# nima-siboni/collectivecrossing

Hardware: NVIDIA B200
Metric: agent_steps_per_sec (higher is better)
Workload: dtype u8 (lattice cells, flag bytes; int32 step counters); rewards: f64 products rounded once to f32

## Files before the change

### __graft_entry__.py

```python

from __future__ import annotations

import sys
from pathlib import Path

ROOT = Path(__file__).resolve().parent
for p in (str(ROOT), str(ROOT / "tests")):
    if p not in sys.path:
        sys.path.insert(0, p)


def build() -> None:
    from collectivecrossing_b200 import _native

    from collectivecrossing_b200 import _abi

    _native.build(force=True)
    lib = _native.library()
    assert lib.cc_abi_version() == _abi.ABI_VERSION
    import oracle
    from oracle import stage_ref

    oracle.build(force=True)
    oracle.lib()
    stage_ref.stage()
    _write_sass()
    import collectivecrossing_b200


def _write_sass() -> None:
    import re
    import subprocess
    from collections import Counter

    from collectivecrossing_b200 import _native

    out_dir = ROOT / "profiles" / "sass"
    out_dir.mkdir(parents=True, exist_ok=True)
    wanted = {"cc_step_tpe2_kernel_8_fp32_b5": r"cc_step_tpe2_kernelILi8ELi4ELi5E", "cc_step_tpe2_kernel_8_int8_b5": r"cc_step_tpe2_kernelILi8ELi1ELi5E",
              "cc_step_tpe2_kernel_8_table_b5": r"cc_step_tpe2_kernelILi8ELi16ELi5E", "cc_step_tpe2_kernel_8_none_b5": r"cc_step_tpe2_kernelILi8ELi0ELi5E",
              "cc_step_tpe_kernel_8_fp32": r"cc_step_tpe_kernelILi8ELi4E", "cc_kernel_32_2_int8_step": r"cc_kernelILi32ELi2ELi1ELi0E"}
    try:
        dump = subprocess.run(["cuobjdump", "-sass", str(_native.LIB_PATH)], capture_output=True, text=True, check=True).stdout
    except Exception as exc:
        print(f"SASS dump skipped: {exc}")
        return
    for stale in out_dir.glob("*.sass"):
        stale.unlink()
    parts = re.split(r"(?=\n\s*Function : )", dump)
    counts = {}
    for name, pat in wanted.items():
        body = next((q for q in parts if re.search(r"Function : \S*" + pat, q)), None)
        if body is None:
            continue
        lines = [f"{m.group(1)}  {m.group(2).strip()}" for m in re.finditer(r"^\s+/\*([0-9a-f]{4,6})\*/\s+(.*?;)\s+/\*", body, flags=re.M)]
        head = body.strip().splitlines()[0]
        (out_dir / f"{name}.sass").write_text(head + "\n" + "\n".join(lines) + "\n")
        ops = Counter(re.sub(r"^@!?U?P\w+\s+", "", ln.split("  ", 1)[1]).split()[0].rstrip(";") for ln in lines)
        counts[name] = {"instructions": sum(ops.values()), "top": dict(ops.most_common(25)),
                        "tma": {k: v for k, v in ops.items() if k.startswith(("UBLKCP", "UTMA", "SYNCS"))}}
    import json

    (out_dir / "mnemonic_counts.json").write_text(json.dumps(counts, indent=1) + "\n")
    log = ROOT / "collectivecrossing_b200" / "csrc" / "ptxas.log"
    if log.exists():
        rows, name = [], None
        for ln in log.read_text().splitlines():
            m = re.search(r"Function properties for (\S+)", ln)
            if m:
                name = m.group(1)
            elif name and "bytes stack frame" in ln:
                stack = ln.strip()
            elif name and "Used" in ln and "registers" in ln:
                rows.append(f"{name}\n    {ln.split(':', 1)[1].strip()}; {stack}")
                name = None
        (out_dir / "ptxas_summary.txt").write_text("\n".join(sorted(set(rows))) + "\n")


def smoke() -> None:
    import numpy as np
    import torch
    from cases import readme_config

    import oracle
    from collectivecrossing_b200 import BatchedCollectiveCrossing, _abi
    from collectivecrossing_b200.lowering import lower_config

    cfg = readme_config(max_steps=20)
    n = 2048
    env = BatchedCollectiveCrossing(cfg, n, "cuda:0", seed=3, obs_dtype="float32", auto_reset=True, with_info=True)
    orc = oracle.OracleEnvs(lower_config(cfg), n, seed=3)
    env.reset()
    orc.reset()
    for t in range(30):
        out = env.step(policy="greedy")
        res = orc.step(policy="greedy", auto_reset=True, obs_dtype=_abi.OBS_FP32)
    torch.cuda.synchronize()
    env.check_error()
    assert np.array_equal(env.x.cpu().numpy(), orc.x) and np.array_equal(env.y.cpu().numpy(), orc.y)
    assert np.array_equal(env.flags.cpu().numpy(), orc.flags) and np.array_equal(env.step_count.cpu().numpy(), orc.step_count)
    assert np.array_equal(out.obs.cpu().numpy(), res["obs"]) and np.array_equal(out.reward.cpu().numpy(), res["reward"])
    assert np.array_equal(out.agent_flags.cpu().numpy(), res["agent_flags"]) and np.array_equal(out.env_flags.cpu().numpy(), res["env_flags"])
    st = env.stats()
    assert st["episodes"] == orc.stats.episodes > 0
    traj = env.rollout_trajectory(8, policy="greedy")
    for t in range(8):
        res = orc.step(policy="greedy", auto_reset=True, obs_dtype=_abi.OBS_FP32)
        assert np.array_equal(traj["obs"][t].cpu().numpy(), res["obs"]) and np.array_equal(traj["reward"][t].cpu().numpy(), res["reward"])
        assert np.array_equal(traj["agent_flags"][t].cpu().numpy(), res["agent_flags"]) and np.array_equal(traj["env_flags"][t].cpu().numpy(), res["env_flags"])
    assert np.array_equal(env.x.cpu().numpy(), orc.x) and np.array_equal(env.flags.cpu().numpy(), orc.flags)
    env.set_host_expand(2)
    host = env.make_host_buffers()
    env.step_host(host, policy="greedy")
    res = orc.step(policy="greedy", auto_reset=True, obs_dtype=_abi.OBS_FP32)
    assert np.array_equal(host["obs"].numpy(), res["obs"]) and np.array_equal(host["reward"].numpy(), res["reward"])
    assert np.array_equal(host["env_flags"].numpy(), res["env_flags"]) and env.last_host_call()["expand_threads"] == 1
    env.check_error()
    print(f"smoke ok: {n} envs x 39 steps, {st['episodes']} episodes, {env.launch_count} kernel launches "
          f"({env.last_kernel} mapping), bit-exact vs oracle")


if __name__ == "__main__":
# ... 3 lines not shown
```

### collectivecrossing_b200/csrc/cc_kernel_tpe2.cuh

```cuda
#pragma once
#include "cc_kernel_tpe.cuh"

#ifndef CCB_T2_MIN_BLOCKS
#define CCB_T2_MIN_BLOCKS 6
#endif

namespace ccb {

constexpr int kT2Warps = 4;
constexpr int kT2Threads = kT2Warps * 32;
constexpr int kT2MaxRows = 16, kT2MaxCols = 32, kT2MaxCells = 256;
constexpr int kT2BitmapBytesPerWarp = kT2MaxRows * 128;

enum { kT2InTram = 1u << 5, kT2AtDoor = 1u << 6, kT2Arrived = 1u << 7, kT2Valid = 1u << 28, kT2SpawnExcluded = 1u << 29 };

struct T2Tables {
    uint2 tab[2 * kT2MaxCells];
    uint8_t act2[kPolicyRows * 16];
    int dcell[8];
};
static_assert(sizeof(T2Tables) % 16 == 0, "copied as 16-byte vectors");

template <int A, int OBS>
struct T2Layout {
    static constexpr bool kImage = OBS == CC_OBS_INT8;
    static constexpr int kEnvBytes = A * (6 + 4 * A);
    static constexpr int kImageBytes = kImage ? 32 * kEnvBytes : 0;
    using L1 = TpeLayout<A, CC_OBS_FP32>;
    static constexpr bool kRows32 = OBS == CC_OBS_FP32;
    static constexpr int kRows32Bytes = kRows32 ? L1::kStageBytesPerWarp : 0;
    static constexpr bool kDirtyBitmap = kImage || kRows32;
    static constexpr int kBitmapOffset = kRows32 ? L1::kTplBytesPerWarp : 0;
    static constexpr int kBytesNeeded = kImage ? kImageBytes : (kRows32 ? kRows32Bytes : 0);
    static constexpr int kBytesPerWarp = kBytesNeeded > kBitmapOffset + kT2BitmapBytesPerWarp ? kBytesNeeded : kBitmapOffset + kT2BitmapBytesPerWarp;
    static constexpr int kDynBytes = kT2Warps * kBytesPerWarp;
};

__device__ __forceinline__ unsigned t2_fill(unsigned w, int k) {
    unsigned r;
    asm("prmt.b32 %0, %1, %2, %3;" : "=r"(r) : "r"(w), "r"(0u), "r"(0x8888u | ((unsigned)k * 0x1111u)));
    return r;
}
template <int B>
__device__ __forceinline__ unsigned t2_gather4(unsigned a, unsigned b, unsigned c, unsigned d) {
    const unsigned lo = __byte_perm(a, b, (unsigned)(B | ((4 + B) << 4)));
    const unsigned hi = __byte_perm(c, d, (unsigned)(B | ((4 + B) << 4)));
    return __byte_perm(lo, hi, 0x5410u);
}
template <int A, int B>
__device__ __forceinline__ void t2_gather(const uint2 (&e)[A], unsigned (&w)[2]) {
    auto g = [&](int k) { return e[k < A ? k : A - 1].x; };
    w[0] = t2_gather4<B>(g(0), g(1), g(2), g(3));
    w[1] = A > 4 ? t2_gather4<B>(g(4), g(5), g(6), g(7)) : 0u;
}
template <int A, bool STREAM>
__device__ __forceinline__ void t2_store_packed(void *base, int env, unsigned w0, unsigned w1) {
    unsigned char *q = static_cast<unsigned char *>(base) + (size_t)env * A;
    if constexpr (A == 8) {
        if constexpr (STREAM) __stcs(reinterpret_cast<uint2 *>(q), make_uint2(w0, w1));
        else *reinterpret_cast<uint2 *>(q) = make_uint2(w0, w1);
    } else if constexpr (A == 4) {
        if constexpr (STREAM) __stcs(reinterpret_cast<unsigned *>(q), w0);
        else *reinterpret_cast<unsigned *>(q) = w0;
    } else {
#pragma unroll
        for (int k = 0; k < A; ++k) q[k] = (unsigned char)((k < 4 ? w0 : w1) >> (8 * (k & 3)));
    }
}

#ifdef CCB_WITH_T2_TABLES
__global__ void __launch_bounds__(256) cc_t2_tables_kernel(const __grid_constant__ KParams p, T2Tables *out) {
    const int PW = p.W + 3, PH = p.H + 3;
    uint2 *tab = out->tab;
    uint8_t *act2 = out->act2;
    int *dcell = out->dcell;
    for (int i = threadIdx.x; i < 2 * kT2MaxCells; i += blockDim.x) {
        const int cell = i >> 1, type = i & 1;
        const int yy = cell / PW - 1, xx = cell - (yy + 1) * PW - 1;
        unsigned geo = 0;
        float rew = 0.f;
        if (cell < PW * PH && xx >= 0 && xx <= p.W && yy >= 0 && yy <= p.H) {
            const unsigned xv = make_xt(p, xx), yv = make_yt(p, type, yy);
            const unsigned u = xv + yv, f = (xv & yv) >> 24;
            const bool in_tram = f & 1u, at_door = f & 2u, arrived = f & 8u;
            const unsigned right = valid_position(p, xx + 1, yy), up = valid_position(p, xx, yy + 1), left = valid_position(p, xx - 1, yy),
                           down = valid_position(p, xx, yy - 1);
            geo = (u & 31u) | (in_tram ? kT2InTram : 0u) | (at_door ? kT2AtDoor : 0u) | (arrived ? kT2Arrived : 0u) | ((unsigned)xx << 8) |
                  ((unsigned)yy << 16) | ((right | (up << 1) | (left << 2) | (down << 3)) << 20) | ((left | (up << 1) | (right << 2) | (down << 3)) << 24) |
                  (valid_position(p, xx, yy) ? kT2Valid : 0u) | ((p.DL <= xx && xx <= p.DR && yy == p.D - 1) ? kT2SpawnExcluded : 0u);
            const bool boarding = type == 0;
            switch (p.reward_kind) {
            case CC_REWARD_DEFAULT:
                if (arrived) rew = p.rpf[0];
                else if (boarding) rew = at_door ? p.rpf[1] : (in_tram ? p.rpf[2] : (float)((double)(-(abs(xx - p.DC) + (p.D - yy))) * p.rp[3]));
                else rew = !in_tram ? p.rpf[2] : (float)((double)(abs(xx - p.DC) + (yy - p.D)) * p.rp[3]);
                break;
            case CC_REWARD_SIMPLE_DISTANCE: rew = (float)((double)(-abs(yy - (boarding ? p.YB : p.YE))) * p.rp[0]); break;
            case CC_REWARD_BINARY: rew = p.rpf[1]; break;
            default: rew = p.rpf[0]; break;
            }
        } else {
            geo = ((unsigned)min(max(xx, 0), p.W) << 8) | ((unsigned)min(max(yy, 0), p.H) << 16);
        }
        tab[i] = make_uint2(geo, __float_as_uint(rew));
    }
    for (int i = threadIdx.x; i < kPolicyRows * 16; i += blockDim.x) {
        const unsigned m = (unsigned)i & 15u;
        act2[i] = (uint8_t)greedy_decision(i >> 4, ((m >> 2) & 1u) | (m & 2u) | ((m & 1u) << 2) | (m & 8u));
    }
    if (threadIdx.x < 8) dcell[threadIdx.x] = threadIdx.x == 0 ? 1 : (threadIdx.x == 1 ? PW : (threadIdx.x == 2 ? -1 : (threadIdx.x == 3 ? -PW : 0)));
}
#endif

template <int A, int OBS, int BT>
__global__ void __launch_bounds__(kT2Threads, CCB_T2_MIN_BLOCKS) cc_step_tpe2_kernel(const __grid_constant__ KParams p) {
    using L = T2Layout<A, OBS>;
    const int B = BT >= 0 ? BT : p.B;
    static_assert(A >= 1 && A <= 8, "thread-per-env mapping is for crews of at most 8");
    static_assert(OBS == CC_OBS_NONE || OBS == CC_OBS_TABLE || (OBS == CC_OBS_INT8 && A == 8) || (OBS == CC_OBS_FP32 && A % 2 == 0),
                  "int8 rows: 8 agents; float32 rows: even crews (an env's block must be whole 16-byte vectors for the bulk copies)");
    static_assert(!L::kRows32 || L::L1::kTma, "float32 rows leave through the TMA image ring");
    constexpr unsigned kOnes = 0x01010101u;
    constexpr unsigned kM0 = A >= 4 ? kOnes : (kOnes >> (8 * (4 - A)));
    constexpr unsigned kM1 = A <= 4 ? 0u : (A == 8 ? kOnes : (kOnes >> (8 * (8 - A))));
    extern __shared__ __align__(16) unsigned char smem[];
    __shared__ __align__(16) T2Tables tb;
    __shared__ unsigned long long red_all[kT2Warps * kStCount];

    const int lane = threadIdx.x & 31, warp = threadIdx.x >> 5;
    const int PW = p.W + 3, PH = p.H + 3;

    for (int i = threadIdx.x; i < (int)(sizeof(T2Tables) / 16); i += blockDim.x)
        reinterpret_cast<uint4 *>(&tb)[i] = static_cast<const uint4 *>(p.t2_tables)[i];
    const int n_warps = (int)blockDim.x >> 5;
    for (int i = threadIdx.x; i < n_warps * L::kBytesPerWarp / 4; i += blockDim.x) reinterpret_cast<unsigned *>(smem)[i] = 0u;
    __shared__ __align__(16) unsigned lut[L::kRows32 ? L::L1::kLutWords : 4];
    if constexpr (L::kRows32) {
        __syncthreads();
        using L1 = typename L::L1;
        for (int w = threadIdx.x; w < L1::kLutWords; w += blockDim.x) {
            const int src = w < L1::PPE ? tpe_source<A>(w / L1::R, w % L1::R) : kSrcM;
            lut[w] = src >= 0 ? (unsigned)(src * L1::PSZ) : (0x80000000u | (unsigned)(-src));
        }
        float2 *t = reinterpret_cast<float2 *>(smem + warp * L::kBytesPerWarp + lane * L1::TSB);
        t[2 * A] = make_float2((float)p.DC, (float)p.D); t[2 * A + 1] = make_float2((float)p.DL, (float)p.DR); t[2 * A + 2] = make_float2(-1.f, -1.f);
    }
    const TpeConstPairs kc = {make_uint2(__float_as_uint((float)p.DC), __float_as_uint((float)p.D)),
                              make_uint2(__float_as_uint((float)p.DL), __float_as_uint((float)p.DR)),
                              make_uint2(__float_as_uint(-1.f), __float_as_uint(-1.f))};
    unsigned long long *red = red_all + warp * kStCount;
    if (lane < kStCount) red[lane] = 0ull;
    if (blockIdx.x == 0 && threadIdx.x == 0) *p.tpe_counter_next = 0u;
    __syncthreads();

    const unsigned tab_s = (unsigned)__cvta_generic_to_shared(tb.tab), act_s = (unsigned)__cvta_generic_to_shared(tb.act2),
                   dc_s = (unsigned)__cvta_generic_to_shared(tb.dcell);
    unsigned char *wsmem = smem + warp * L::kBytesPerWarp;
    const unsigned img_s = (unsigned)__cvta_generic_to_shared(wsmem);
    const unsigned bm = img_s + (unsigned)L::kBitmapOffset + 4u * lane;
    unsigned tbase[A];
#pragma unroll
    for (int k = 0; k < A; ++k) tbase[k] = tab_s + (k < B ? 0u : 8u);
    unsigned boardw[2];
    boardw[0] = (B >= 4 ? kOnes : (B <= 0 ? 0u : (kOnes >> (8 * (4 - B))))) & kM0;
    boardw[1] = (B <= 4 ? 0u : (B >= 8 ? kOnes : (kOnes >> (8 * (8 - B))))) & kM1;
    const unsigned typew0 = kM0 & ~boardw[0], typew1 = kM1 & ~boardw[1];

    auto lookup = [&](unsigned c, int k) {
        CCB_CHECK(c < (unsigned)kT2MaxCells);
        uint2 e;
        asm volatile("ld.shared.v2.u32 {%0, %1}, [%2];" : "=r"(e.x), "=r"(e.y) : "r"(tbase[k] + c * 16u));
        return e;
    };
    auto lds32 = [&](unsigned addr) { unsigned v; asm volatile("ld.shared.u32 %0, [%1];" : "=r"(v) : "r"(addr)); return v; };
    auto sts32 = [&](unsigned addr, unsigned v) { asm volatile("st.shared.u32 [%0], %1;" ::"r"(addr), "r"(v) : "memory"); };

    unsigned st_arrivals = 0;
    double st_rsum = 0.0;
    int errbits = 0;
    const int total_warps = (int)gridDim.x * n_warps;
    const int n_groups = (int)p.n_groups;
    int gw = (int)blockIdx.x * n_warps + warp;
    int g_next = 0;
    for (; gw < n_groups; gw = g_next) {
        const int g = p.tpe_reverse ? n_groups - 1 - gw : gw;
        const long long nn = (long long)g * 32 + lane;
        const int nl = nn < p.n_envs ? (int)nn : (int)p.n_envs - 1;
        const uint2 xw_in = tpe_fetch_row<A>(p.x, nl), yw_in = tpe_fetch_row<A>(p.y, nl), fw_in = tpe_fetch_row<A>(p.flags, nl);
        int step = p.step[nl];
        float ep_ret = p.ep_ret[nl];
#if CCB_TPE_DYNAMIC
        if (lane == 0) g_next = total_warps + (int)atomicAdd(p.tpe_counter, 1u);
#else
        g_next = gw + total_warps;
#endif
        const int n = g * 32 + lane;
        const int envs_here = (int)min(32ll, p.n_envs - (long long)g * 32);
        const bool env_ok = lane < envs_here;
        const unsigned long long genv = p.genv_offset + (unsigned long long)n;
// ... 148 lines not shown
#pragma unroll
            for (int l = 0; l < LPE; ++l) leaf[l] = l < A ? 0.f + rew[l < A ? l : 0] : 0.f;
#pragma unroll
            for (int w = LPE / 2; w >= 1; w >>= 1)
#pragma unroll
                for (int l = 0; l < w; ++l) leaf[l] = leaf[l] + leaf[l + w];
            rsum = leaf[0];
        }
        ep_ret += rsum;
        const bool done = term_all || trunc_all;
        unsigned eflags = (term_all ? CC_E_TERMINATED_ALL : 0u) | (trunc_all ? CC_E_TRUNCATED_ALL : 0u);

        if (env_ok) {
            float *rw = reinterpret_cast<float *>(p.reward) + slice_a + (size_t)n * A;
            if constexpr (A % 4 == 0) {
#pragma unroll
                for (int k = 0; k < A; k += 4) __stcs(reinterpret_cast<float4 *>(rw + k), make_float4(rew[k], rew[k + 1], rew[k + 2], rew[k + 3]));
            } else {
#pragma unroll
                for (int k = 0; k < A; ++k) rw[k] = rew[k];
            }
            t2_store_packed<A, true>(p.agent_flags + slice_a, n, of0, of1);
            if (p.agent_info) {
                const unsigned i0 = ((fb[0] >> 5) & 0x03030303u) | ((fb[0] >> 4) & 0x08080808u) | ((fl[0] & kOnes) << 2);
                const unsigned i1 = ((fb[1] >> 5) & 0x03030303u) | ((fb[1] >> 4) & 0x08080808u) | ((fl[1] & kOnes) << 2);
                t2_store_packed<A, true>(p.agent_info + slice_a, n, i0 & (kM0 * 15u), i1 & (kM1 * 15u));
            }
            st_rsum += (double)rsum;
        }
        const bool ended = env_ok && done && any_alive;
        const unsigned ended_mask = __ballot_sync(kFull, ended);
        if (ended_mask) {
            const unsigned n_term = __popc(__ballot_sync(kFull, ended && term_all)), n_trunc = __popc(__ballot_sync(kFull, ended && trunc_all));
            unsigned len = ended ? (unsigned)step : 0u;
            double ret = ended ? (double)ep_ret : 0.0;
#pragma unroll
            for (int w = 16; w >= 1; w >>= 1) { len += __shfl_xor_sync(kFull, len, w); ret += __shfl_xor_sync(kFull, ret, w); }
            if (lane == 0) {
                red[kStEpisodes] += __popc(ended_mask); red[kStTermAll] += n_term; red[kStTruncAll] += n_trunc; red[kStEpLen] += len;
                red[kStEpRet] = (unsigned long long)__double_as_longlong(__longlong_as_double((long long)red[kStEpRet]) + ret);
            }
        }

        if (env_ok && done && p.auto_reset) {
            eflags |= CC_E_WAS_RESET;
            ep_ret = 0.f;
            step = 0;
#pragma unroll
            for (int i = 0; i < A; ++i) {
                unsigned cand = 0;
                bool ok = false;
                for (int attempt = 0; attempt < kResetAttemptCap && !ok; ++attempt) {
                    const U4 r = draw_at(p, t_rng, genv, kStreamReset, ((unsigned)i << 16) | (unsigned)attempt);
                    int cx, cy;
                    if (i < B) { cx = bounded(r.v0, p.W); cy = bounded(r.v1, p.D); }
                    else { cx = p.TL + bounded(r.v0, p.TR + 1 - p.TL); cy = p.D + bounded(r.v1, p.H - p.D); }
                    cand = (unsigned)((cy + 1) * PW + cx + 1);
                    CCB_CHECK(cand < (unsigned)(PW * PH));
                    const unsigned ge = tb.tab[(cand & 255u) * 2].x;
                    ok = (ge & kT2Valid) && !(i < B && (ge & kT2SpawnExcluded));
#pragma unroll
                    for (int j = 0; j < i; ++j) ok = ok && c[j] != cand;
                }
                if (!ok) errbits |= kErrResetStuck;
                c[i] = cand & 255u;
            }
            fl[0] = kM0; fl[1] = kM1;
#pragma unroll
            for (int k = 0; k < A; ++k) e[k] = lookup(c[k], k);
            t2_gather<A, 0>(e, fb);
        }
        if (env_ok) __stcs(reinterpret_cast<unsigned char *>(p.env_flags) + (size_t)tt * (size_t)p.slice_envs + n, (unsigned char)eflags);

        if constexpr (OBS == CC_OBS_FP32) {
            using L1 = typename L::L1;
            float2 *tpl = reinterpret_cast<float2 *>(wsmem + lane * L1::TSB);
#pragma unroll
            for (int k = 0; k < A; ++k) {
                tpl[2 * k] = make_float2((float)(int)((e[k].x >> 8) & 0xffu), (float)(int)((e[k].x >> 16) & 0xfu));
                tpl[2 * k + 1] = make_float2(k < B ? 0.f : 1.f, (float)(int)(((k < 4 ? fl[0] : fl[1]) >> (8 * (k & 3))) & 1u));
            }
            __syncwarp();
            void *obs_t = static_cast<unsigned char *>(p.obs) + (size_t)tt * (size_t)p.slice_obs_bytes;
            tpe_emit_group_tma<A, CC_OBS_FP32>(lut, img_s, obs_t, g, envs_here, lane, kc);
            __syncwarp();
        } else if constexpr (OBS != CC_OBS_NONE) {
            unsigned T[A];
#pragma unroll
            for (int k = 0; k < A; ++k)
                T[k] = ((e[k].x >> 8) & 0x0fffu) | ((((k < 4 ? typew0 : typew1) >> (8 * (k & 3))) & 1u) << 16) | ((((k < 4 ? fl[0] : fl[1]) >> (8 * (k & 3))) & 1u) << 24);
            if constexpr (OBS == CC_OBS_TABLE) {
                if (env_ok) {
                    unsigned *dst = reinterpret_cast<unsigned *>(static_cast<unsigned char *>(p.obs) + (size_t)tt * (size_t)p.slice_obs_bytes) + (size_t)n * A;
                    if constexpr (A % 4 == 0) {
#pragma unroll
                        for (int k = 0; k < A; k += 4) __stcs(reinterpret_cast<uint4 *>(dst + k), make_uint4(T[k], T[k + 1], T[k + 2], T[k + 3]));
                    } else {
#pragma unroll
                        for (int k = 0; k < A; ++k) __stcs(dst + k, T[k]);
                    }
                }
            } else {
                if (lane == 0) asm volatile("cp.async.bulk.wait_group.read 0;" ::: "memory");
                __syncwarp();
                const unsigned K1 = (unsigned)(p.DC & 0xff) | ((unsigned)(p.D & 0xff) << 8), K2 = (unsigned)(p.DL & 0xff) | ((unsigned)(p.DR & 0xff) << 8);
                const unsigned KK = K1 | (K2 << 16);
                unsigned S[7];
#pragma unroll
                for (int j = 0; j < 7; ++j) S[j] = __byte_perm(T[j], T[j + 1], 0x5432u);
                unsigned wv[76];
#pragma unroll
                for (int m = 0; m < 4; ++m) {
                    const int a = 2 * m, b = 2 * m + 1;
                    unsigned *w = wv + 19 * m;
                    w[0] = (T[a] & 0xffffu) | (K1 << 16);
                    w[1] = K2 | ((a == 0 ? 0xffffu : (T[0] & 0xffffu)) << 16);
#pragma unroll
                    for (int j = 0; j < 7; ++j) w[2 + j] = (j == a - 1) ? (S[j] | 0xffff0000u) : ((j == a) ? (S[j] | 0x0000ffffu) : S[j]);
                    w[9] = (a == 7 ? 0xffffu : (T[7] >> 16)) | (T[b] << 16);
                    w[10] = KK;
#pragma unroll
                    for (int j = 0; j < 8; ++j) w[11 + j] = j == b ? 0xffffffffu : T[j];
                }
                const unsigned dst_s = img_s + (unsigned)lane * (unsigned)L::kEnvBytes;
                CCB_CHECK(dst_s + 19u * 16u <= img_s + (unsigned)L::kBytesPerWarp && envs_here * L::kEnvBytes <= L::kImageBytes && (envs_here * L::kEnvBytes) % 16 == 0);
#pragma unroll
                for (int v = 0; v < 19; ++v)
                    asm volatile("st.shared.v4.u32 [%0], {%1, %2, %3, %4};" ::"r"(dst_s + 16u * v), "r"(wv[4 * v]), "r"(wv[4 * v + 1]), "r"(wv[4 * v + 2]), "r"(wv[4 * v + 3]) : "memory");
                asm volatile("fence.proxy.async.shared::cta;" ::: "memory");
                __syncwarp();
                if (lane == 0) {
                    unsigned char *dst = static_cast<unsigned char *>(p.obs) + (size_t)tt * (size_t)p.slice_obs_bytes + (size_t)g * 32 * L::kEnvBytes;
                    unsigned long long l2_evict_first;
                    asm volatile("createpolicy.fractional.L2::evict_first.b64 %0, 1.0;" : "=l"(l2_evict_first));
                    asm volatile("cp.async.bulk.global.shared::cta.bulk_group.L2::cache_hint [%0], [%1], %2, %3;"
                                 ::"l"(dst), "r"(img_s), "r"((unsigned)(envs_here * L::kEnvBytes)), "l"(l2_evict_first) : "memory");
                    asm volatile("cp.async.bulk.commit_group;" ::: "memory");
                }
            }
        }
      }

        if (env_ok) {
            unsigned xw[2], yw[2];
            t2_gather<A, 1>(e, xw);
            t2_gather<A, 2>(e, yw);
            t2_store_packed<A, false>(p.x, n, xw[0], xw[1]);
            t2_store_packed<A, false>(p.y, n, yw[0] & 0x0f0f0f0fu, yw[1] & 0x0f0f0f0fu);
            t2_store_packed<A, false>(p.flags, n, fl[0], fl[1]);
            p.step[n] = step;
            p.ep_ret[n] = ep_ret;
        }
#if CCB_TPE_DYNAMIC
        g_next = __shfl_sync(kFull, g_next, 0);
#endif
    }

    if (L::kDirtyBitmap && lane == 0) asm volatile("cp.async.bulk.wait_group 0;" ::: "memory");
    {
        double rs = st_rsum;
        unsigned ar = st_arrivals;
#pragma unroll
        for (int w = 16; w >= 1; w >>= 1) { rs += __shfl_xor_sync(kFull, rs, w); ar += __shfl_xor_sync(kFull, ar, w); }
        if (lane == 0) {
            red[kStArrivals] += ar;
            red[kStRewardSum] = (unsigned long long)__double_as_longlong(rs);
        }
// ... 19 lines not shown
```

### collectivecrossing_b200/csrc/cc_launch_tpe.cu

```cuda
#include <cstdio>
#include <cstdlib>

#if CCB_TPE_PART == 1
#define CCB_WITH_T2_TABLES 1
#endif
#include "cc_internal.h"
#include "cc_kernel_tpe2.cuh"

#ifndef CCB_TPE_PART
#error "compile with -DCCB_TPE_PART=0 (crews 1-4 and 8-agent int8 rows) or 1 (crews 5-8)"
#endif

namespace {

using ccb::KParams;

template <int A, int OBS>
int launch_tpe_t(cc_handle *h, KParams p, cudaStream_t s) {
    using L = ccb::TpeLayout<A, OBS>;
    auto kern = ccb::cc_step_tpe_kernel<A, OBS>;
    p.n_groups = (p.n_envs + 31) / 32;
    const bool on_device_policy = p.policy == CC_POLICY_GREEDY || p.policy == CC_POLICY_WAITING;
    const int bm_cap = L::kTma ? (L::kImgRing * L::kImgBytes / 128 < ccb::kTpeMaxBitmapWords ? L::kImgRing * L::kImgBytes / 128 : ccb::kTpeMaxBitmapWords)
                               : ccb::kTpeMaxBitmapWords;
    p.tpe_bm_words = (on_device_policy && p.walk_words <= bm_cap) ? p.walk_words : 0;
    if (on_device_policy && p.W + 3 <= 32 && p.H + 3 <= bm_cap) { p.tpe_bm_words = p.H + 3; p.tpe_bm_rows = 1; }
    if (p.n_steps < 1) p.n_steps = 1;
    p.tpe_counter = h->tpe_counters + (h->tpe_launches & 1);
    p.tpe_counter_next = h->tpe_counters + ((h->tpe_launches + 1) & 1);
    const int smem = L::kStageBytes + (L::kTma ? 0 : p.tpe_bm_words * ccb::kTpeThreads * 4);
    int per_sm = 0;
    int rc = cc_cached_occupancy(h, reinterpret_cast<const void *>(kern), ccb::kTpeThreads, smem, &per_sm);
    if (rc != CC_OK) return rc;
    long long want = (p.n_groups + ccb::kTpeWarps - 1) / ccb::kTpeWarps;
    long long cap = (long long)h->sm_count * per_sm;
    int grid = (int)(want < cap ? want : cap);
    if (grid < 1) grid = 1;
    kern<<<grid, ccb::kTpeThreads, smem, s>>>(p);
    CC_CUDA(cudaGetLastError());
    snprintf(h->last_kernel, sizeof h->last_kernel, "ccb::cc_step_tpe_kernel<%d,%d>", A, OBS);
    h->launches += 1;
    h->tpe_launches += 1;
    return CC_OK;
}

template <int A, int OBS, int BT = -1>
int launch_tpe2_t(cc_handle *h, KParams p, cudaStream_t s) {
    using L = ccb::T2Layout<A, OBS>;
    auto kern = ccb::cc_step_tpe2_kernel<A, OBS, BT>;
    int rc0 = cc_t2_ensure_tables(h, p, s);
    if (rc0 != CC_OK) return rc0;
    p.t2_tables = h->t2_tables;
    p.n_groups = (p.n_envs + 31) / 32;
    if (p.n_steps < 1) p.n_steps = 1;
    p.tpe_counter = h->tpe_counters + (h->tpe_launches & 1);
    p.tpe_counter_next = h->tpe_counters + ((h->tpe_launches + 1) & 1);
    int warps = ccb::kT2Warps;
    int per_sm = 0;
    int rc = cc_cached_occupancy(h, reinterpret_cast<const void *>(kern), warps * 32, warps * L::kBytesPerWarp, &per_sm);
    if (rc != CC_OK) return rc;
    if (p.n_groups <= (long long)h->sm_count * per_sm * warps) {
        warps = 2;
        rc = cc_cached_occupancy(h, reinterpret_cast<const void *>(kern), warps * 32, warps * L::kBytesPerWarp, &per_sm);
        if (rc != CC_OK) return rc;
    }
    const int smem = warps * L::kBytesPerWarp;
    long long want = (p.n_groups + warps - 1) / warps;
    long long cap = (long long)h->sm_count * per_sm;
    int grid = (int)(want < cap ? want : cap);
    if (grid < 1) grid = 1;
    kern<<<grid, warps * 32, smem, s>>>(p);
    CC_CUDA(cudaGetLastError());
    snprintf(h->last_kernel, sizeof h->last_kernel, "ccb::cc_step_tpe2_kernel<%d,%d>", A, OBS);
    h->launches += 1;
    h->tpe_launches += 1;
    return CC_OK;
}

bool tpe2_eligible(const KParams &p, int obs_dtype) {
    static const bool enabled = [] { const char *v = std::getenv("CCB200_TPE2"); return !(v && v[0] == '0'); }();
    const int PW = p.W + 3, PH = p.H + 3;
    static const bool rows32 = [] { const char *v = std::getenv("CCB200_TPE2_FP32"); return !(v && v[0] == '0'); }();
    if (obs_dtype == CC_OBS_FP32 && (!rows32 || p.A % 2 != 0)) return false;
    return enabled && PW <= ccb::kT2MaxCols && PH <= ccb::kT2MaxRows && PW * PH <= ccb::kT2MaxCells;
}

}

#define CCB_TPE2_CASES(A_)                                                                  \
    case A_ * 32 + CC_OBS_NONE: return launch_tpe2_t<A_, CC_OBS_NONE>(h, p, s);                 \
    case A_ * 32 + CC_OBS_TABLE: return launch_tpe2_t<A_, CC_OBS_TABLE>(h, p, s);
#define CCB_TPE2_CASES_EVEN(A_)                                                             \
    CCB_TPE2_CASES(A_)                                                                      \
    case A_ * 32 + CC_OBS_FP32: return launch_tpe2_t<A_, CC_OBS_FP32>(h, p, s);
#define CCB_TPE_CASES(A_)                                                                   \
    case A_ * 32 + CC_OBS_NONE: return launch_tpe_t<A_, CC_OBS_NONE>(h, p, s);                  \
    case A_ * 32 + CC_OBS_TABLE: return launch_tpe_t<A_, CC_OBS_TABLE>(h, p, s);                \
    case A_ * 32 + CC_OBS_FP32: return launch_tpe_t<A_, CC_OBS_FP32>(h, p, s);

#if CCB_TPE_PART == 0
int cc_launch_tpe_part0(cc_handle *h, const KParams &p, int obs_dtype, cudaStream_t s) {
    if (tpe2_eligible(p, obs_dtype)) {
        switch (p.A * 32 + obs_dtype) { CCB_TPE2_CASES(1) CCB_TPE2_CASES_EVEN(2) CCB_TPE2_CASES(3) CCB_TPE2_CASES_EVEN(4) }
    }
    switch (p.A * 32 + obs_dtype) {
        CCB_TPE_CASES(1) CCB_TPE_CASES(2) CCB_TPE_CASES(3) CCB_TPE_CASES(4)
    case 8 * 32 + CC_OBS_INT8: return launch_tpe_t<8, CC_OBS_INT8>(h, p, s);
    }
    return cc_fail(CC_ERR_UNSUPPORTED, "no thread-per-env kernel for %d agents, obs_dtype %d", p.A, obs_dtype);
}
#else
int cc_launch_tpe_part0(cc_handle *h, const KParams &p, int obs_dtype, cudaStream_t s);
int cc_t2_ensure_tables(cc_handle *h, const KParams &p, cudaStream_t s) {
    if (h->t2_tables) return CC_OK;
    void *buf = nullptr;
    cudaError_t e = cudaMalloc(&buf, sizeof(ccb::T2Tables));
    if (e != cudaSuccess) return cc_fail(CC_ERR_NOMEM, "cudaMalloc for the small-lattice tables: %s", cudaGetErrorString(e));
    ccb::cc_t2_tables_kernel<<<1, 256, 0, s>>>(p, static_cast<ccb::T2Tables *>(buf));
    e = cudaGetLastError();
    if (e != cudaSuccess) { cudaFree(buf); return cc_fail(CC_ERR_CUDA, "cc_t2_tables_kernel: %s", cudaGetErrorString(e)); }
    h->t2_tables = buf;
    return CC_OK;
}

int cc_launch_tpe(cc_handle *h, const KParams &p, int obs_dtype, cudaStream_t s) {
    if (tpe2_eligible(p, obs_dtype)) {
        if (p.A == 8 && p.B == 5) {
            switch (obs_dtype) {
            case CC_OBS_NONE: return launch_tpe2_t<8, CC_OBS_NONE, 5>(h, p, s);
            case CC_OBS_TABLE: return launch_tpe2_t<8, CC_OBS_TABLE, 5>(h, p, s);
            case CC_OBS_INT8: return launch_tpe2_t<8, CC_OBS_INT8, 5>(h, p, s);
            case CC_OBS_FP32: return launch_tpe2_t<8, CC_OBS_FP32, 5>(h, p, s);
            }
        }
        switch (p.A * 32 + obs_dtype) {
            CCB_TPE2_CASES(5) CCB_TPE2_CASES_EVEN(6) CCB_TPE2_CASES(7) CCB_TPE2_CASES_EVEN(8)
        case 8 * 32 + CC_OBS_INT8: return launch_tpe2_t<8, CC_OBS_INT8>(h, p, s);
        }
    }
    switch (p.A * 32 + obs_dtype) {
        CCB_TPE_CASES(5) CCB_TPE_CASES(6) CCB_TPE_CASES(7) CCB_TPE_CASES(8)
    }
    return cc_launch_tpe_part0(h, p, obs_dtype, s);
}
#endif
```

### profiles/probes/tma_ring_probe.cu

```cuda
#include <cstdio>
#include <cstdint>
#include <cuda_runtime.h>

constexpr int kChunkBytes = 38912;
constexpr int kThreads = 256;

template <int IMG, int RING, bool COMPUTE, int SMALL = 0>
__global__ void __launch_bounds__(kThreads) probe(unsigned char *out, int n_chunks, int *counter, int chase_len, unsigned *sink, unsigned char *small = nullptr) {
    __shared__ unsigned tab[1024];
    extern __shared__ __align__(128) unsigned char dyn[];
    const int lane = threadIdx.x & 31, warp = threadIdx.x >> 5;
    for (int i = threadIdx.x; i < 1024; i += blockDim.x) tab[i] = i * 7919u + 13u;
    __syncthreads();
    const uint2 v = make_uint2(1, threadIdx.x);
    if ((SMALL & 64) && threadIdx.x < 5) {
        const size_t N = (size_t)n_chunks * 32;
        const size_t bytes = threadIdx.x < 3 ? N * 8 : N * 4;
        const unsigned char *base = threadIdx.x < 3 ? small + threadIdx.x * N * 8 : small + 3 * N * 8 + (threadIdx.x - 3) * N * 4;
        const size_t share = ((bytes + gridDim.x - 1) / gridDim.x + 15) / 16 * 16;
        const size_t lo = (size_t)blockIdx.x * share;
        if (lo < bytes) {
            const size_t len = lo + share <= bytes ? share : bytes - lo;
            for (size_t o = 0; o < len; o += 16384) {
                const unsigned sz = (unsigned)(len - o < 16384 ? len - o : 16384);
// ... 22 lines not shown
                r += *reinterpret_cast<const unsigned *>(srec + 768 + lane * 4) + *reinterpret_cast<const unsigned *>(srec + 896 + lane * 4);
                acc += (unsigned)r;
                for (int a = 0; a < 3; ++a) *reinterpret_cast<unsigned long long *>(srec + a * 256 + lane * 8) = r + a;
                *reinterpret_cast<unsigned *>(srec + 768 + lane * 4) = acc;
                *reinterpret_cast<unsigned *>(srec + 896 + lane * 4) = acc + 1;
                reinterpret_cast<uint4 *>(orec)[2 * lane] = make_uint4(acc, 1, 2, 3);
                reinterpret_cast<uint4 *>(orec)[2 * lane + 1] = make_uint4(acc, 1, 2, 3);
                for (int a = 0; a < 3; ++a) *reinterpret_cast<unsigned long long *>(orec + 1024 + a * 256 + lane * 8) = r + a;
                orec[1792 + lane] = (unsigned char)acc;
            } else {
            auto ld8 = [&](const void *q) { unsigned long long v;
                if (SMALL & 8) asm volatile("ld.global.L2::cache_hint.u64 %0, [%1], %2;" : "=l"(v) : "l"(q), "l"(pol_last));
                else v = *reinterpret_cast<const unsigned long long *>(q);
                return v; };
            auto st8 = [&](void *q, unsigned long long v) {
                if (SMALL & 8) asm volatile("st.global.L2::cache_hint.u64 [%0], %1, %2;" ::"l"(q), "l"(v), "l"(pol_last) : "memory");
                else *reinterpret_cast<unsigned long long *>(q) = v; };
            if (SMALL & 1) {
                for (int a = 0; a < 3; ++a) r += ld8(small + a * N * 8 + n * 8);
                r += ld8(small + 3 * N * 8 + (n / 2) * 8);
                r += ld8(small + 3 * N * 8 + N * 4 + (n / 2) * 8);
            }
            acc += (unsigned)r;
            if (SMALL & 2) {
                for (int a = 0; a < 3; ++a) st8(small + a * N * 8 + n * 8, r + a);
                reinterpret_cast<unsigned *>(small + 3 * N * 8)[n] = acc;
                reinterpret_cast<unsigned *>(small + 3 * N * 8 + N * 4)[n] = acc + 1;
            }
            if (SMALL & 4) {
                for (int a = 4; a < 7; ++a) *reinterpret_cast<unsigned long long *>(small + a * N * 8 + n * 8) = r + a;
                reinterpret_cast<uint4 *>(small + 7 * N * 8)[2 * n] = make_uint4(acc, 1, 2, 3);
                reinterpret_cast<uint4 *>(small + 7 * N * 8)[2 * n + 1] = make_uint4(acc, 1, 2, 3);
                small[11 * N * 8 + n] = (unsigned char)acc;
            }
            }
        }
        for (int b = 0; b < kChunkBytes / IMG; ++b) {
            if (lane == 0) asm volatile("cp.async.bulk.wait_group.read %0;" ::"n"(RING - 1) : "memory");
            __syncwarp();
            uint2 *s = reinterpret_cast<uint2 *>(ring + buf * IMG) + lane;
#pragma unroll
            for (int j = 0; j < (IMG + 255) / 256; ++j)
                if (j * 256 + 256 <= IMG || lane * 8 + j * 256 < IMG) s[32 * j] = v;
            asm volatile("fence.proxy.async.shared::cta;" ::: "memory");
            __syncwarp();
            if (lane == 0) {
                unsigned char *dst = out + (long long)g * kChunkBytes + b * IMG;
                const unsigned src = (unsigned)__cvta_generic_to_shared(ring + buf * IMG);
                if (SMALL & 16) {
                    unsigned long long pf;
                    asm volatile("createpolicy.fractional.L2::evict_first.b64 %0, 1.0;" : "=l"(pf));
                    asm volatile("cp.async.bulk.global.shared::cta.bulk_group.L2::cache_hint [%0], [%1], %2, %3;" ::"l"(dst), "r"(src), "n"(IMG), "l"(pf) : "memory");
                } else
                asm volatile("cp.async.bulk.global.shared::cta.bulk_group [%0], [%1], %2;" ::"l"(dst), "r"(src), "n"(IMG) : "memory");
                asm volatile("cp.async.bulk.commit_group;" ::: "memory");
            }
            buf = buf + 1 == RING ? 0 : buf + 1;
        }
    }
    if (lane == 0) asm volatile("cp.async.bulk.wait_group 0;" ::: "memory");
    sink[blockIdx.x * blockDim.x + threadIdx.x] = acc;
}

template <int IMG, int RING, bool COMPUTE, int SMALL = 0>
void run(unsigned char *out, int *counter, unsigned *sink, int sms, int cps, int chase_len, unsigned char *small = nullptr) {
    const int n_chunks = 32768, dyn = 8 * RING * IMG;
    auto kern = probe<IMG, RING, COMPUTE, SMALL>;
    cudaFuncSetAttribute(kern, cudaFuncAttributeMaxDynamicSharedMemorySize, dyn);
    cudaEvent_t e0, e1; cudaEventCreate(&e0); cudaEventCreate(&e1);
    float best = 1e9;
    for (int rep = 0; rep < 6; ++rep) {
        cudaMemsetAsync(counter, 0, 4);
        cudaEventRecord(e0);
        kern<<<sms * cps, kThreads, dyn>>>(out, n_chunks, counter, chase_len, sink, small);
        cudaEventRecord(e1); cudaEventSynchronize(e1);
        float ms; cudaEventElapsedTime(&ms, e0, e1);
        if (rep >= 2 && ms < best) best = ms;
    }
    printf("side traffic mode %2d, image %5d B x ring %d (%6d B in flight per warp), %d CTAs/SM, compute %d: %8.4f ms %7.1f GB/s (%s)\n", SMALL, IMG, RING, IMG * RING, cps,
           (int)COMPUTE, best, 32768.0 * kChunkBytes / 1e9 / (best * 1e-3), cudaGetErrorString(cudaGetLastError()));
    fflush(stdout);
}

int main() {
    unsigned char *out; cudaMalloc(&out, (size_t)32768 * kChunkBytes);
    int *counter; cudaMalloc(&counter, 4);
    unsigned *sink; cudaMalloc(&sink, 4 * 148 * 8 * kThreads);
    int sms; cudaDeviceGetAttribute(&sms, cudaDevAttrMultiProcessorCount, 0);
    const int chase = 600;
    unsigned char *small; cudaMalloc(&small, (size_t)32768 * 32 * 8 * 12); cudaMemset(small, 0, (size_t)32768 * 32 * 8 * 12);
    {
        cudaDeviceProp prop; cudaGetDeviceProperties(&prop, 0);
        printf("L2 %d MB, persistingL2CacheMaxSize %d MB, accessPolicyMaxWindowSize %d MB\n", prop.l2CacheSize >> 20, prop.persistingL2CacheMaxSize >> 20, prop.accessPolicyMaxWindowSize >> 20);
    }
    run<1216, 2, false, 0>(out, counter, sink, sms, 3, 0, small);
    run<1216, 2, false, 1>(out, counter, sink, sms, 3, 0, small);
    run<1216, 2, false, 2>(out, counter, sink, sms, 3, 0, small);
    run<1216, 2, false, 3>(out, counter, sink, sms, 3, 0, small);
    run<1216, 2, false, 4>(out, counter, sink, sms, 3, 0, small);
    run<1216, 2, false, 7>(out, counter, sink, sms, 3, 0, small);
    run<1216, 2, false, 7 + 8>(out, counter, sink, sms, 3, 0, small);
    run<1216, 2, false, 7 + 16>(out, counter, sink, sms, 3, 0, small);
    run<1216, 2, false, 7 + 8 + 16>(out, counter, sink, sms, 3, 0, small);
    run<1216, 2, false, 1 + 32>(out, counter, sink, sms, 3, 0, small);
    run<1216, 2, false, 7 + 32>(out, counter, sink, sms, 3, 0, small);
    run<1216, 2, false, 6>(out, counter, sink, sms, 3, 0, small);
    run<1216, 2, false, 6 + 32>(out, counter, sink, sms, 3, 0, small);
    for (size_t carve_mb : {36, 48, 64}) {
        cudaDeviceSetLimit(cudaLimitPersistingL2CacheSize, carve_mb << 20);
        cudaStreamAttrValue attr = {};
        attr.accessPolicyWindow.base_ptr = small;
        attr.accessPolicyWindow.num_bytes = (size_t)32 << 20;
        attr.accessPolicyWindow.hitRatio = 1.0f;
        attr.accessPolicyWindow.hitProp = cudaAccessPropertyPersisting;
        attr.accessPolicyWindow.missProp = cudaAccessPropertyNormal;
        cudaError_t e = cudaStreamSetAttribute(0, cudaStreamAttributeAccessPolicyWindow, &attr);
        printf("state window 32 MB persisting, carve-out %zu MB: %s\n", carve_mb, cudaGetErrorString(e));
        run<1216, 2, false, 3>(out, counter, sink, sms, 3, 0, small);
        run<1216, 2, false, 7>(out, counter, sink, sms, 3, 0, small);
        run<1216, 2, false, 7 + 16>(out, counter, sink, sms, 3, 0, small);
        attr.accessPolicyWindow.num_bytes = 0;
        cudaStreamSetAttribute(0, cudaStreamAttributeAccessPolicyWindow, &attr);
        cudaCtxResetPersistingL2Cache();
    }
    cudaDeviceSetLimit(cudaLimitPersistingL2CacheSize, 0);
    run<1216, 2, false, 7>(out, counter, sink, sms, 3, 0, small);
    return 0;
    run<1216, 2, false, 128>(out, counter, sink, sms, 3, 0, small);
    run<1216, 2, false, 128 + 16>(out, counter, sink, sms, 3, 0, small);
    run<1216, 2, true, 128 + 16>(out, counter, sink, sms, 3, 100, small);
    run<1216, 2, false, 1 + 64>(out, counter, sink, sms, 3, 0, small);
    run<1216, 2, false, 7 + 64>(out, counter, sink, sms, 3, 0, small);
    run<1216, 2, false, 7 + 16 + 64>(out, counter, sink, sms, 3, 0, small);
    run<1216, 2, true, 7 + 16 + 64>(out, counter, sink, sms, 3, 100, small);
    run<1216, 2, true, 7 + 16>(out, counter, sink, sms, 3, 100, small);
    return 0;
    {
        cudaDeviceProp prop; cudaGetDeviceProperties(&prop, 0);
        for (size_t win_mb : {32, 64, 97}) {
            size_t carve = (size_t)prop.persistingL2CacheMaxSize;
            cudaDeviceSetLimit(cudaLimitPersistingL2CacheSize, carve);
            cudaStreamAttrValue attr = {};
            attr.accessPolicyWindow.base_ptr = small;
            attr.accessPolicyWindow.num_bytes = win_mb << 20;
            attr.accessPolicyWindow.hitRatio = 1.0f;
            attr.accessPolicyWindow.hitProp = cudaAccessPropertyPersisting;
            attr.accessPolicyWindow.missProp = cudaAccessPropertyStreaming;
            cudaError_t e = cudaStreamSetAttribute(0, cudaStreamAttributeAccessPolicyWindow, &attr);
            printf("persisting window %zu MB (carve-out %zu MB): %s\n", win_mb, carve >> 20, cudaGetErrorString(e));
            run<1216, 2, false, 7>(out, counter, sink, sms, 3, 0, small);
            run<1216, 2, false, 7 + 16>(out, counter, sink, sms, 3, 0, small);
            run<1216, 2, true, 7 + 16>(out, counter, sink, sms, 3, 100, small);
        }
        cudaStreamAttrValue attr = {};
        attr.accessPolicyWindow.num_bytes = 0;
        cudaStreamSetAttribute(0, cudaStreamAttributeAccessPolicyWindow, &attr);
        cudaCtxResetPersistingL2Cache();
    }
    return 0;
    for (int cps : {3}) {
        run<1216, 2, false>(out, counter, sink, sms, cps, chase);
        run<1216, 2, true>(out, counter, sink, sms, cps, chase);
        run<1216, 4, true>(out, counter, sink, sms, cps, chase);
        run<2432, 2, true>(out, counter, sink, sms, cps, chase);
        run<4864, 2, true>(out, counter, sink, sms, cps, chase);
        run<9728, 2, true>(out, counter, sink, sms, cps, chase);
        run<4864, 1, true>(out, counter, sink, sms, cps, chase);
// ... 4 lines not shown
```

Before: 43.29 billion.

## Batch eight env observation images per TMA bulk store in fp32 tpe2 path

For 8-agent float32 observations, the tpe2 kernel now stages eight environments' images contiguously in a two-slot shared-memory ring and issues one larger cp.async.bulk store per group of eight, instead of one bulk copy per environment. The aim is to cut the number of bulk-copy issues and waits and to make global writes larger. In exchange, shared memory per warp grows, which may lower the min-blocks occupancy bound (now derived from the smem budget). A probe benchmark sweeping images-per-copy and ring depth was added.

```diff
diff --git a/__graft_entry__.py b/__graft_entry__.py
--- a/__graft_entry__.py
+++ b/__graft_entry__.py
@@ -37,7 +37,7 @@
 
     out_dir = ROOT / "profiles" / "sass"
     out_dir.mkdir(parents=True, exist_ok=True)
-    wanted = {"cc_step_tpe2_kernel_8_fp32_b5": r"cc_step_tpe2_kernelILi8ELi4ELi5E", "cc_step_tpe2_kernel_8_int8_b5": r"cc_step_tpe2_kernelILi8ELi1ELi5E",
+    wanted = {"cc_step_tpe2_kernel_8_fp32_b5": r"cc_step_tpe2_kernelILi8ELi4ELi5ELi8E", "cc_step_tpe2_kernel_8_int8_b5": r"cc_step_tpe2_kernelILi8ELi1ELi5E",
               "cc_step_tpe2_kernel_8_table_b5": r"cc_step_tpe2_kernelILi8ELi16ELi5E", "cc_step_tpe2_kernel_8_none_b5": r"cc_step_tpe2_kernelILi8ELi0ELi5E",
               "cc_step_tpe_kernel_8_fp32": r"cc_step_tpe_kernelILi8ELi4E", "cc_kernel_32_2_int8_step": r"cc_kernelILi32ELi2ELi1ELi0E"}
     try:
diff --git a/collectivecrossing_b200/csrc/cc_kernel_tpe2.cuh b/collectivecrossing_b200/csrc/cc_kernel_tpe2.cuh
--- a/collectivecrossing_b200/csrc/cc_kernel_tpe2.cuh
+++ b/collectivecrossing_b200/csrc/cc_kernel_tpe2.cuh
@@ -21,20 +21,78 @@
 };
 static_assert(sizeof(T2Tables) % 16 == 0, "copied as 16-byte vectors");
 
-template <int A, int OBS>
+template <int A, int OBS, int IE = 1>
 struct T2Layout {
     static constexpr bool kImage = OBS == CC_OBS_INT8;
     static constexpr int kEnvBytes = A * (6 + 4 * A);
     static constexpr int kImageBytes = kImage ? 32 * kEnvBytes : 0;
     using L1 = TpeLayout<A, CC_OBS_FP32>;
     static constexpr bool kRows32 = OBS == CC_OBS_FP32;
-    static constexpr int kRows32Bytes = kRows32 ? L1::kStageBytesPerWarp : 0;
+    static constexpr int kImgEnvs = IE, kImgRing = IE == 1 ? L1::kImgRing : 2;
+    static constexpr int kImgBytes = kImgEnvs * L1::kImgBytes;
+    static constexpr int kRows32Bytes = kRows32 ? L1::kTplBytesPerWarp + kImgRing * kImgBytes : 0;
     static constexpr bool kDirtyBitmap = kImage || kRows32;
     static constexpr int kBitmapOffset = kRows32 ? L1::kTplBytesPerWarp : 0;
     static constexpr int kBytesNeeded = kImage ? kImageBytes : (kRows32 ? kRows32Bytes : 0);
     static constexpr int kBytesPerWarp = kBytesNeeded > kBitmapOffset + kT2BitmapBytesPerWarp ? kBytesNeeded : kBitmapOffset + kT2BitmapBytesPerWarp;
     static constexpr int kDynBytes = kT2Warps * kBytesPerWarp;
+    static_assert(IE == 1 || (kRows32 && 32 % IE == 0), "multi-env images: float32 rows, a group is a whole number of images");
+    static constexpr int kSmemBlocks = 233472 / (kDynBytes + 6528);
+    static constexpr int kMinBlocks = IE > 1 && kSmemBlocks < CCB_T2_MIN_BLOCKS ? kSmemBlocks : CCB_T2_MIN_BLOCKS;
 };
+
+template <int A, int IE>
+__device__ __forceinline__ void t2_emit_rows(const unsigned *lut, unsigned sbase, void *obs, int g, int envs_here, int lane) {
+    using L = T2Layout<A, CC_OBS_FP32, IE>;
+    using L1 = typename L::L1;
+    constexpr int E = L::kImgEnvs, RING = L::kImgRing, kImages = 32 / E;
+    unsigned src[L1::kImgInstr];
+#pragma unroll
+    for (int j = 0; j < L1::kImgInstr; ++j) {
+        const unsigned d = lut[j * 32 + lane];
+        src[j] = sbase + ((d >> 31) ? (unsigned)((2 * A - 1 + (int)(d & 3u)) * L1::PSZ) : d);
+    }
+    const unsigned img0 = sbase + L1::kTplBytesPerWarp;
+    const unsigned islot = img0 + 8u * lane;
+    unsigned char *dst = static_cast<unsigned char *>(obs) + (size_t)g * 32 * L1::kImgBytes;
+    unsigned long long l2_evict_first;
+    asm volatile("createpolicy.fractional.L2::evict_first.b64 %0, 1.0;" : "=l"(l2_evict_first));
+    if (lane == 0) asm volatile("cp.async.bulk.wait_group.read 0;" ::: "memory");
+    for (int i0 = 0; i0 < kImages; i0 += RING) {
+#pragma unroll
+        for (int r = 0; r < RING; ++r) {
+            const int e0 = (i0 + r) * E;
+            if (i0 + r >= kImages || e0 >= envs_here) break;
+            if (lane == 0) asm volatile("cp.async.bulk.wait_group.read %0;" ::"n"(RING - 1) : "memory");
+            __syncwarp();
+#pragma unroll
+            for (int k = 0; k < E; ++k) {
+                const unsigned t_off = (unsigned)((r * E + k) * L1::TSB), i_off = (unsigned)(r * L::kImgBytes + k * L1::kImgBytes);
+#pragma unroll
+                for (int j = 0; j < L1::kImgInstr; ++j) {
+                    CCB_CHECK(src[j] + t_off >= sbase && src[j] + t_off + 8u <= sbase + (unsigned)L1::kTplBytesPerWarp);
+                    unsigned long long v;
+                    asm volatile("ld.shared.b64 %0, [%1];" : "=l"(v) : "r"(src[j] + t_off));
+                    if (j * 32 + 32 <= L1::PPE || lane + j * 32 < L1::PPE) {
+                        CCB_CHECK(islot + i_off + 256u * j + 8u <= img0 + (unsigned)(RING * L::kImgBytes));
+                        asm volatile("st.shared.b64 [%0], %1;" ::"r"(islot + i_off + 256u * j), "l"(v) : "memory");
+                    }
+                }
+            }
+            asm volatile("fence.proxy.async.shared::cta;" ::: "memory");
+            __syncwarp();
+            const unsigned bytes = (unsigned)(min(E, envs_here - e0) * L1::kImgBytes);
+            CCB_CHECK(bytes > 0u && bytes <= (unsigned)L::kImgBytes && bytes % 16u == 0u && (reinterpret_cast<uintptr_t>(dst + (size_t)e0 * L1::kImgBytes) & 15) == 0);
+            if (lane == 0) {
+                asm volatile("cp.async.bulk.global.shared::cta.bulk_group.L2::cache_hint [%0], [%1], %2, %3;"
+                             ::"l"(dst + (size_t)e0 * L1::kImgBytes), "r"(img0 + (unsigned)(r * L::kImgBytes)), "r"(bytes), "l"(l2_evict_first) : "memory");
+                asm volatile("cp.async.bulk.commit_group;" ::: "memory");
+            }
+        }
+#pragma unroll
+        for (int j = 0; j < L1::kImgInstr; ++j) src[j] += (unsigned)(RING * E * L1::TSB);
+    }
+}
 
 __device__ __forceinline__ unsigned t2_fill(unsigned w, int k) {
     unsigned r;
@@ -112,9 +170,9 @@
 }
 #endif
 
-template <int A, int OBS, int BT>
-__global__ void __launch_bounds__(kT2Threads, CCB_T2_MIN_BLOCKS) cc_step_tpe2_kernel(const __grid_constant__ KParams p) {
-    using L = T2Layout<A, OBS>;
+template <int A, int OBS, int BT, int IE = 1>
+__global__ void __launch_bounds__(kT2Threads, T2Layout<A, OBS, IE>::kMinBlocks) cc_step_tpe2_kernel(const __grid_constant__ KParams p) {
+    using L = T2Layout<A, OBS, IE>;
     const int B = BT >= 0 ? BT : p.B;
     static_assert(A >= 1 && A <= 8, "thread-per-env mapping is for crews of at most 8");
     static_assert(OBS == CC_OBS_NONE || OBS == CC_OBS_TABLE || (OBS == CC_OBS_INT8 && A == 8) || (OBS == CC_OBS_FP32 && A % 2 == 0),
@@ -429,7 +487,8 @@
             }
             __syncwarp();
             void *obs_t = static_cast<unsigned char *>(p.obs) + (size_t)tt * (size_t)p.slice_obs_bytes;
-            tpe_emit_group_tma<A, CC_OBS_FP32>(lut, img_s, obs_t, g, envs_here, lane, kc);
+            if constexpr (IE == 1) tpe_emit_group_tma<A, CC_OBS_FP32>(lut, img_s, obs_t, g, envs_here, lane, kc);
+            else t2_emit_rows<A, IE>(lut, img_s, obs_t, g, envs_here, lane);
             __syncwarp();
         } else if constexpr (OBS != CC_OBS_NONE) {
             unsigned T[A];
diff --git a/collectivecrossing_b200/csrc/cc_launch_tpe.cu b/collectivecrossing_b200/csrc/cc_launch_tpe.cu
--- a/collectivecrossing_b200/csrc/cc_launch_tpe.cu
+++ b/collectivecrossing_b200/csrc/cc_launch_tpe.cu
@@ -44,6 +44,22 @@
     return CC_OK;
 }
 
+template <int A, int OBS, int BT, int IE>
+int launch_tpe2_grid(cc_handle *h, const KParams &p, cudaStream_t s, int warps, int per_sm) {
+    using L = ccb::T2Layout<A, OBS, IE>;
+    const int smem = warps * L::kBytesPerWarp;
+    long long want = (p.n_groups + warps - 1) / warps;
+    long long cap = (long long)h->sm_count * per_sm;
+    int grid = (int)(want < cap ? want : cap);
+    if (grid < 1) grid = 1;
+    ccb::cc_step_tpe2_kernel<A, OBS, BT, IE><<<grid, warps * 32, smem, s>>>(p);
+    CC_CUDA(cudaGetLastError());
+    snprintf(h->last_kernel, sizeof h->last_kernel, "ccb::cc_step_tpe2_kernel<%d,%d>", A, OBS);
+    h->launches += 1;
+    h->tpe_launches += 1;
+    return CC_OK;
+}
+
 template <int A, int OBS, int BT = -1>
 int launch_tpe2_t(cc_handle *h, KParams p, cudaStream_t s) {
     using L = ccb::T2Layout<A, OBS>;
@@ -63,18 +79,14 @@
         warps = 2;
         rc = cc_cached_occupancy(h, reinterpret_cast<const void *>(kern), warps * 32, warps * L::kBytesPerWarp, &per_sm);
         if (rc != CC_OK) return rc;
+    } else if constexpr (OBS == CC_OBS_FP32 && A == 8) {
+        constexpr int kIE = 8;
+        auto kern8 = ccb::cc_step_tpe2_kernel<A, OBS, BT, kIE>;
+        rc = cc_cached_occupancy(h, reinterpret_cast<const void *>(kern8), warps * 32, warps * ccb::T2Layout<A, OBS, kIE>::kBytesPerWarp, &per_sm);
+        if (rc != CC_OK) return rc;
+        return launch_tpe2_grid<A, OBS, BT, kIE>(h, p, s, warps, per_sm);
     }
-    const int smem = warps * L::kBytesPerWarp;
-    long long want = (p.n_groups + warps - 1) / warps;
-    long long cap = (long long)h->sm_count * per_sm;
-    int grid = (int)(want < cap ? want : cap);
-    if (grid < 1) grid = 1;
-    kern<<<grid, warps * 32, smem, s>>>(p);
-    CC_CUDA(cudaGetLastError());
-    snprintf(h->last_kernel, sizeof h->last_kernel, "ccb::cc_step_tpe2_kernel<%d,%d>", A, OBS);
-    h->launches += 1;
-    h->tpe_launches += 1;
-    return CC_OK;
+    return launch_tpe2_grid<A, OBS, BT, 1>(h, p, s, warps, per_sm);
 }
 
 bool tpe2_eligible(const KParams &p, int obs_dtype) {
diff --git a/profiles/probes/tma_ring_probe.cu b/profiles/probes/tma_ring_probe.cu
--- a/profiles/probes/tma_ring_probe.cu
+++ b/profiles/probes/tma_ring_probe.cu
@@ -128,7 +128,107 @@
     fflush(stdout);
 }
 
-int main() {
+constexpr int kFusedT = 20, kFusedEnvBytes = 1216, kFusedSide = 49, kFusedTpl = 4864;
+
+template <int E, int RING>
+__global__ void __launch_bounds__(128) fused_probe(unsigned char *out, unsigned char *side, int n_groups, int *counter, unsigned *sink) {
+    constexpr int IMG = E * kFusedEnvBytes;
+    extern __shared__ __align__(128) unsigned char dyn[];
+    const int lane = threadIdx.x & 31, warp = threadIdx.x >> 5;
+    unsigned char *ring = dyn + warp * (kFusedTpl + RING * IMG) + kFusedTpl;
+    const size_t N = (size_t)n_groups * 32;
+    const uint2 v = make_uint2(1, threadIdx.x);
+    unsigned long long pf;
+    asm volatile("createpolicy.fractional.L2::evict_first.b64 %0, 1.0;" : "=l"(pf));
+    for (;;) {
+        int g = 0;
+        if (lane == 0) g = atomicAdd(counter, 1);
+        g = __shfl_sync(0xffffffffu, g, 0);
+        if (g >= n_groups) break;
+        const size_t n = (size_t)g * 32 + lane;
+        for (int t = 0; t < kFusedT; ++t) {
+            float4 *rw = reinterpret_cast<float4 *>(side + (size_t)t * N * kFusedSide) + 2 * n;
+            __stcs(rw, make_float4(1.f, 2.f, 3.f, (float)t)); __stcs(rw + 1, make_float4(1.f, 2.f, 3.f, (float)t));
+            __stcs(reinterpret_cast<uint2 *>(side + (size_t)t * N * kFusedSide + N * 32) + n, v);
+            __stcs(reinterpret_cast<uint2 *>(side + (size_t)t * N * kFusedSide + N * 40) + n, v);
+            __stcs(side + (size_t)t * N * kFusedSide + N * 48 + n, (unsigned char)t);
+            if (lane == 0) asm volatile("cp.async.bulk.wait_group.read 0;" ::: "memory");
+            for (int i = 0; i < 32 / E; ++i) {
+                const int buf = i % RING;
+                if (lane == 0) asm volatile("cp.async.bulk.wait_group.read %0;" ::"n"(RING - 1) : "memory");
+                __syncwarp();
+                uint2 *s = reinterpret_cast<uint2 *>(ring + buf * IMG) + lane;
+#pragma unroll
+                for (int j = 0; j < (IMG + 255) / 256; ++j)
+                    if (j * 256 + 256 <= IMG || lane * 8 + j * 256 < IMG) s[32 * j] = v;
+                asm volatile("fence.proxy.async.shared::cta;" ::: "memory");
+                __syncwarp();
+                if (lane == 0) {
+                    unsigned char *dst = out + (size_t)t * N * kFusedEnvBytes + ((size_t)g * 32 + i * E) * kFusedEnvBytes;
+                    const unsigned src = (unsigned)__cvta_generic_to_shared(ring + buf * IMG);
+                    asm volatile("cp.async.bulk.global.shared::cta.bulk_group.L2::cache_hint [%0], [%1], %2, %3;" ::"l"(dst), "r"(src), "n"(IMG), "l"(pf) : "memory");
+                    asm volatile("cp.async.bulk.commit_group;" ::: "memory");
+                }
+            }
+        }
+    }
+    if (lane == 0) asm volatile("cp.async.bulk.wait_group 0;" ::: "memory");
+    sink[blockIdx.x * blockDim.x + threadIdx.x] = v.y;
+}
+
+template <int E, int RING>
+void run_fused(unsigned char *out, unsigned char *side, int n_groups, int *counter, unsigned *sink, int sms, int warps_per_sm) {
+    const int cps = warps_per_sm / 4, dyn = 4 * (kFusedTpl + RING * E * kFusedEnvBytes);
+    auto kern = fused_probe<E, RING>;
+    cudaFuncSetAttribute(kern, cudaFuncAttributeMaxDynamicSharedMemorySize, dyn);
+    int fit = 0;
+    cudaOccupancyMaxActiveBlocksPerMultiprocessor(&fit, kern, 128, dyn);
+    if (fit < cps) {
+        printf("fused T=%d, image %5d B (E=%d) x ring %d, %2d warps/SM: does not fit (%d CTAs of %d B)\n", kFusedT, E * kFusedEnvBytes, E, RING, warps_per_sm, fit, dyn);
+        return;
+    }
+    cudaEvent_t e0, e1; cudaEventCreate(&e0); cudaEventCreate(&e1);
+    float best = 1e9;
+    for (int rep = 0; rep < 6; ++rep) {
+        cudaMemsetAsync(counter, 0, 4);
+        cudaEventRecord(e0);
+        kern<<<sms * cps, 128, dyn>>>(out, side, n_groups, counter, sink);
+        cudaEventRecord(e1); cudaEventSynchronize(e1);
+        float ms; cudaEventElapsedTime(&ms, e0, e1);
+        if (rep >= 2 && ms < best) best = ms;
+    }
+    const double bytes = (double)kFusedT * n_groups * 32 * (kFusedEnvBytes + kFusedSide);
+    printf("fused T=%d, image %5d B (E=%d) x ring %d, %2d warps/SM: %8.4f ms per launch, %7.4f ms per env-step %7.1f GB/s (%s)\n", kFusedT, E * kFusedEnvBytes, E, RING,
+           warps_per_sm, best, best / kFusedT, bytes / 1e9 / (best * 1e-3), cudaGetErrorString(cudaGetLastError()));
+    fflush(stdout);
+}
+
+template <int E, int RING>
+void sweep_fused(unsigned char *out, unsigned char *side, int n_groups, int *counter, unsigned *sink, int sms) {
+    for (int w : {8, 12, 16, 20}) run_fused<E, RING>(out, side, n_groups, counter, sink, sms, w);
+}
+
+int main(int argc, char **argv) {
+    if (argc > 1 && argv[1][0] == 'f') {
+        const int n_groups = 32768;
+        const size_t N = (size_t)n_groups * 32;
+        unsigned char *out, *side; int *counter; unsigned *sink;
+        cudaMalloc(&out, (size_t)kFusedT * N * kFusedEnvBytes);
+        cudaMalloc(&side, (size_t)kFusedT * N * kFusedSide);
+        cudaMalloc(&counter, 4);
+        cudaMalloc(&sink, 4 * 148 * 8 * 128);
+        int sms; cudaDeviceGetAttribute(&sms, cudaDevAttrMultiProcessorCount, 0);
+        sweep_fused<1, 2>(out, side, n_groups, counter, sink, sms);
+        sweep_fused<1, 3>(out, side, n_groups, counter, sink, sms);
+        sweep_fused<2, 2>(out, side, n_groups, counter, sink, sms);
+        sweep_fused<2, 3>(out, side, n_groups, counter, sink, sms);
+        sweep_fused<4, 2>(out, side, n_groups, counter, sink, sms);
+        sweep_fused<4, 3>(out, side, n_groups, counter, sink, sms);
+        sweep_fused<8, 2>(out, side, n_groups, counter, sink, sms);
+        sweep_fused<8, 3>(out, side, n_groups, counter, sink, sms);
+        sweep_fused<1, 2>(out, side, n_groups, counter, sink, sms);
+        return cudaDeviceSynchronize() != cudaSuccess;
+    }
     unsigned char *out; cudaMalloc(&out, (size_t)32768 * kChunkBytes);
     int *counter; cudaMalloc(&counter, 4);
     unsigned *sink; cudaMalloc(&sink, 4 * 148 * 8 * kThreads);
```

After: 44.33 billion, median of 6. +2.4%, better.
